# rubiruchi/ofdm_uhd

Hardware: AMD Instinct MI355X
Metric: OFDM symbols/sec (TX+loopback RX) @ N_fft=512; packet CRC pass rate (higher is better)
Workload: dtype f32; 1 GPU; N_fft=512, occ=200, QPSK, CP=128, synthetic AWGN channel (BASELINE configs[1]); payload_bytes=1026, symbols_per_packet=22, streams=1, iq_buffers=1, parallelism=independent streams, 1 per GPU

## Files before the change

include/ofdm_hip.h:

```cpp
#ifndef OFDM_HIP_H
#define OFDM_HIP_H

#include <stddef.h>
#include <stdint.h>

#ifdef __cplusplus
extern "C" {
#endif

#define OFDM_ABI_VERSION 6

#define OFDM_MAX_FFT 4096
#define OFDM_MAX_CARRIER_HEX 1024
#define OFDM_MAX_TAPS 512
#define OFDM_MAX_ARITY 256
#define OFDM_MASK_LEN 4096
#define OFDM_MAX_PKT_LEN 4096

enum {
  OFDM_OK = 0,
  OFDM_E_INVAL = -1,
  OFDM_E_NOMEM = -2,
  OFDM_E_CAPACITY = -3,
  OFDM_E_HIP = -4,
// ... 441 lines not shown
  OFDM_K_CHAN = 2,
  OFDM_K_SYNC = 3,
  OFDM_K_PEAK = 4,
  OFDM_K_DEMOD = 5,
  OFDM_K_DEFRAME = 6,
  OFDM_K_SENSE = 7,
  OFDM_K_FILTER = 8,
  OFDM_K_EXACT = 9,
  OFDM_K_FRONT = 10,
  OFDM_K_COUNT = 11
};
int ofdm_prof_enable(ofdm_handle *h, int on);
int ofdm_prof_reset(ofdm_handle *h);
int ofdm_prof_get(ofdm_handle *h, int kernel, double *total_ms, uint64_t *launches);
const char *ofdm_kernel_name(int kernel);

#ifdef __cplusplus
}
#endif
#endif
```

ofdm_uhd_amd/_abi.py:

```python
import ctypes as C
import os

OFDM_ABI_VERSION = 6
OFDM_MAX_FFT = 4096
OFDM_MAX_TAPS = 512
OFDM_MAX_ARITY = 256
OFDM_MASK_LEN = 4096
OFDM_MAX_PKT_LEN = 4096
OFDM_MAX_CARRIER_HEX = 1024
OFDM_DDC_MAX_TAPS = 1024
OFDM_DDC_BANK_MAX_LINKS = 8
OFDM_RESAMP_MAX_TAPS = 1024
OFDM_RESAMP_BANK_MAX_LINKS = 8
OFDM_DUC_MAX_TAPS = 1024
OFDM_DUC_BANK_MAX_LINKS = 8
OFDM_TX_RESAMP_MAX_TAPS = 1024
OFDM_TX_RESAMP_BANK_MAX_LINKS = 8
OFDM_PFB_MAX_CHANNELS = 64
OFDM_PFB_MAX_TAPS = 1024
OFDM_MULTIPATH_MAX_PATHS = 16
OFDM_MULTIPATH_MAX_TONES = 4
OFDM_MULTIPATH_MAX_DELAY = 1023
OFDM_FEC_MAX_PAYLOAD = 2040
OFDM_FEC_MAX_CODED = 4090
# ... 262 lines not shown
    ]


class ofdm_soft_cfg(C.Structure):
    _fields_ = [
        ("struct_size", C.c_uint32),
        ("scale", C.c_float),
    ]


EXPORTS = (
    "ofdm_abi_version", "ofdm_device_count", "ofdm_create", "ofdm_destroy", "ofdm_last_error",
    "ofdm_set_stream", "ofdm_set_tx_amplitude", "ofdm_set_carrier_map", "ofdm_set_channel", "ofdm_framed_len",
    "ofdm_make_packets", "ofdm_tx_frame_count", "ofdm_tx", "ofdm_tx_async", "ofdm_wait", "ofdm_channel", "ofdm_rx",
    "ofdm_set_taps", "ofdm_tap", "ofdm_prof_enable", "ofdm_prof_reset", "ofdm_prof_get",
    "ofdm_kernel_name", "ofdm_sense_count", "ofdm_sense", "ofdm_sense_decide", "ofdm_set_rx_sense",
    "ofdm_rx_sense_result", "ofdm_sense_device_msgs", "ofdm_sense_redecide",
    "ofdm_rx_packet_pos", "ofdm_rx_nco_state", "ofdm_rx_set_flag_history", "ofdm_rx_set_origin", "ofdm_rx_submit", "ofdm_rx_snr",
    "ofdm_set_rx_quality", "ofdm_rx_quality", "ofdm_set_rx_csi", "ofdm_rx_csi", "ofdm_rx_csi_summary",
    "ofdm_set_rx_iq_format", "ofdm_set_tx_iq_format",
    "ofdm_set_ddc", "ofdm_ddc_reset", "ofdm_ddc_count", "ofdm_ddc", "ofdm_ddc_taps", "ofdm_ddc_last_ms",
    "ofdm_set_duc", "ofdm_duc_reset", "ofdm_duc", "ofdm_duc_last_ms",
    "ofdm_set_ddc_bank", "ofdm_ddc_bank_reset", "ofdm_ddc_bank_count", "ofdm_ddc_bank", "ofdm_ddc_bank_taps",
    "ofdm_ddc_bank_last_ms",
    "ofdm_set_resamp", "ofdm_resamp_reset", "ofdm_resamp_count", "ofdm_resamp", "ofdm_resamp_taps", "ofdm_resamp_last_ms",
    "ofdm_set_resamp_bank", "ofdm_resamp_bank_reset", "ofdm_resamp_bank_count", "ofdm_resamp_bank", "ofdm_resamp_bank_taps",
    "ofdm_resamp_bank_last_ms",
    "ofdm_set_tx_resamp", "ofdm_tx_resamp_reset", "ofdm_tx_resamp_count", "ofdm_tx_resamp", "ofdm_tx_resamp_last_ms",
    "ofdm_set_pfb", "ofdm_pfb_reset", "ofdm_pfb_count", "ofdm_pfb", "ofdm_pfb_last_ms",
    "ofdm_set_pfb_synth", "ofdm_pfb_synth_reset", "ofdm_pfb_synth", "ofdm_pfb_synth_last_ms",
    "ofdm_set_duc_bank", "ofdm_duc_bank_reset", "ofdm_duc_bank", "ofdm_duc_bank_taps", "ofdm_duc_bank_last_ms",
# ... 101 lines not shown
    lib.ofdm_fec_last_ms.argtypes = [H, C.POINTER(C.c_double)]
    lib.ofdm_fec_coded_len_rate.argtypes = [C.c_uint32, C.c_uint32, u32p]
    lib.ofdm_fec_payload_len_rate.argtypes = [C.c_uint32, C.c_uint32, u32p]
    lib.ofdm_fec_punct_last_ms.argtypes = [H, C.POINTER(C.c_double)]
    lib.ofdm_set_rx_soft.argtypes = [H, C.POINTER(ofdm_soft_cfg)]
    lib.ofdm_rx_soft.argtypes = [H, vp, C.c_uint64, u64p, C.POINTER(C.c_int)]
    lib.ofdm_rx_fec_decode_soft.argtypes = [H, FC, u8p, C.c_uint64, u64p, vp, u32p, C.c_int, C.POINTER(C.c_int)]
    lib.ofdm_rx_soft_last_ms.argtypes = [H, C.POINTER(C.c_double)]
    lib.ofdm_set_taps.argtypes = [H, C.c_uint32]
    lib.ofdm_tap.argtypes = [H, C.c_int, vp, C.c_uint64, u64p]
    lib.ofdm_prof_enable.argtypes = [H, C.c_int]
    lib.ofdm_prof_reset.argtypes = [H]
    lib.ofdm_prof_get.argtypes = [H, C.c_int, C.POINTER(C.c_double), u64p]
    lib.ofdm_kernel_name.argtypes = [C.c_int]
    lib.ofdm_kernel_name.restype = C.c_char_p
    SC = C.POINTER(ofdm_sense_cfg)
    lib.ofdm_sense_count.argtypes = [SC, C.c_uint64, u64p, u64p]
    lib.ofdm_sense.argtypes = [H, SC, vp, C.c_uint64, vp, C.c_uint64, vp, vp, vp, C.c_uint64, u64p, u64p]
    lib.ofdm_sense_decide.argtypes = [H, SC, vp, C.c_uint64, vp, vp, vp, C.c_uint64, u64p]
    lib.ofdm_set_rx_sense.argtypes = [H, SC]
    lib.ofdm_rx_sense_result.argtypes = [H, vp, C.c_uint64, vp, vp, vp, C.c_uint64, u64p, u64p]
    lib.ofdm_rx_packet_pos.argtypes = [H, vp, C.c_int, C.POINTER(C.c_int)]
    lib.ofdm_rx_nco_state.argtypes = [H, vp, vp, vp, vp, C.c_int, C.POINTER(C.c_int)]
    lib.ofdm_rx_set_origin.argtypes = [H, C.c_uint64]
    lib.ofdm_rx_snr.argtypes = [H, C.POINTER(C.c_float)]
    lib.ofdm_set_rx_quality.argtypes = [H, C.c_int]
    lib.ofdm_rx_quality.argtypes = [H, vp, C.c_int, C.POINTER(C.c_int)]
    lib.ofdm_set_rx_csi.argtypes = [H, C.c_int]
    lib.ofdm_rx_csi.argtypes = [H, C.c_int, C.c_int, vp, vp, vp, vp, C.POINTER(C.c_int)]
    lib.ofdm_rx_csi_summary.argtypes = [H, C.c_int, u32p, vp, vp, vp, vp, vp]
# ... 39 lines not shown
```

ofdm_uhd_amd/csrc/engine.hip:

```cpp
#include <math.h>
#include <cmath>
#include <stdlib.h>
#include <string.h>

#include <algorithm>
#include <new>
#include <string>
#include <vector>

#include "common.h"
#include "fft.h"
#include "host_util.h"
#include "tx.h"
#include "rx_sync.h"
#include "rx_demod.h"
#include "rx_deframe.h"
#include "rx_soft.h"
#include "rx_state.h"
#include "sense.h"
#include "stream_hist.h"
#include "ddc.h"
#include "ddc_bank.h"
#include "duc.h"
#include "duc_bank.h"
// ... 287 lines not shown
  h->cfg.carrier_map[OFDM_MAX_CARRIER_HEX + 7] = 0;
  {
    int rc = apply_carrier_map(h, h->cfg.carrier_map);
    if (rc != OFDM_OK) return rc;
  }

  std::vector<c32> pre(N), tw(N);
  for (int i = 0; i < N; i++) pre[i] = c32{0.f, 0.f};
  for (int i = 0; i < occ; i++) {
    if (h->zl + i < N) pre[h->zl + i] = c32{cfg->known_symbol[i].re, cfg->known_symbol[i].im};
  }
  for (int k = 0; k < N; k++) {
    double a = -2.0 * M_PI * (double)k / (double)N;
    tw[k] = c32{(float)cos(a), (float)sin(a)};
  }
  uint32_t crc[256];
  for (uint32_t i = 0; i < 256; i++) {
    uint32_t c = i;
    for (int k = 0; k < 8; k++) c = (c & 1) ? (0xEDB88320u ^ (c >> 1)) : (c >> 1);
    crc[i] = c;
  }
  h->filtF = sync_filter_F((int)cfg->ntaps);
  std::vector<c32> Hf(h->filtF), twF(h->filtF);
  {
    const int F = h->filtF;
    std::vector<double> cs(F), sn(F);
    for (int m = 0; m < F; m++) {
      const double a = -2.0 * M_PI * (double)m / (double)F;
      cs[m] = cos(a);
      sn[m] = sin(a);
      twF[m] = c32{(float)cs[m], (float)sn[m]};
    }
    for (int k = 0; k < F; k++) {
      double re = 0.0, im = 0.0;
      for (int n = 0; n < (int)cfg->ntaps; n++) {
        const int idx = (int)(((long long)k * n) % F);
// ... 72 lines not shown
        if (seen & (1 << ix)) ok4 = false;
        seen |= 1 << ix;
        h->sign_idx[ix] = (unsigned char)i;
      }
      if (ok4) h->sign_kind = 2;
    }
    if (h->sign_kind) {
      const float lvl = h->sign_kind == 1 ? fabsf(c[0].re) : fminf(fabsf(c[0].re), fabsf(c[0].im));
      h->sign_eps = lvl * (1.0f / 512.0f);
      h->sign_bound = 8.0f * fmaxf(fabsf(c[0].re), fabsf(c[0].im));
    }
  }
  HIPCHK(h, upload(h->d_preamble, pre.data(), pre.size()));
  HIPCHK(h, upload(h->d_tw, tw.data(), tw.size()));
  HIPCHK(h, upload(h->d_mask, cfg->whitening_mask, (size_t)OFDM_MASK_LEN));
  HIPCHK(h, upload(h->d_crc, crc, (size_t)256));
  {
    std::vector<uint32_t> xp8(OFDM_MASK_LEN + 1);
    uint32_t v = 0x80000000u;
    for (size_t k = 0; k < xp8.size(); k++) {
      xp8[k] = v;
      for (int b = 0; b < 8; b++) v = (v & 1u) ? ((v >> 1) ^ 0xEDB88320u) : (v >> 1);
    }
    HIPCHK(h, upload(h->d_xp8, xp8.data(), xp8.size()));
  }
  {
    const double decay = (double)(1.0f - cfg->peak_alpha);
    std::vector<double> tab(2 * (SYNC_TILE + 1) + SYNC_THREADS / 2);
    double* dp = tab.data();
    double* ip = dp + (SYNC_TILE + 1);
    float* wt = reinterpret_cast<float*>(ip + (SYNC_TILE + 1));
// ... 495 lines not shown
```

ofdm_uhd_amd/csrc/engine_rx.inc:

```

template <typename T>
static int dev_excl_scan(ofdm_handle* h, const T* d_in, uint64_t n, T* d_out, T* d_total) {
  const uint64_t nb = (n + SCAN_BLOCK - 1) / SCAN_BLOCK;
  HIPCHK(h, h->rx.partial.ensure(sizeof(T) * std::max<uint64_t>(nb, 1)));
  T* part = h->rx.partial.as<T>();
  if (n == 0) {
    if (d_total) HIPCHK(h, hipMemsetAsync(d_total, 0, sizeof(T), h->stream));
    return OFDM_OK;
  }
  hipLaunchKernelGGL(HIP_KERNEL_NAME(k_scan_partials<T>), dim3((unsigned)nb), dim3(256), 0, h->stream, d_in, n, part);
  hipLaunchKernelGGL(HIP_KERNEL_NAME(k_scan_top<T>), dim3(1), dim3(256), 0, h->stream, part, nb, d_total);
  hipLaunchKernelGGL(HIP_KERNEL_NAME(k_scan_final<T>), dim3((unsigned)nb), dim3(256), 0, h->stream, d_in, n, part, d_out);
  HIPCHK(h, hipGetLastError());
  return OFDM_OK;
}

template <int N, bool TWL, bool TAPS, bool CSI = false>
static int launch_demod_t(ofdm_handle* h, const DemodParams& q, size_t shmem) {
  constexpr int T = N / 8, FPW = demod_fpw(N);
  if (shmem > 64 * 1024)
    HIPCHK(h, hipFuncSetAttribute(reinterpret_cast<const void*>(&k_rx_demod<N, TWL, TAPS, CSI>),
                                  hipFuncAttributeMaxDynamicSharedMemorySize, (int)shmem));
  hipLaunchKernelGGL(HIP_KERNEL_NAME(k_rx_demod<N, TWL, TAPS, CSI>), dim3((q.nframes + FPW - 1) / FPW), dim3(T * FPW), shmem,
                     h->stream, q);
// ... 38 lines not shown
}

static int run_demod(ofdm_handle* h, const DemodParams& q) {
  switch (h->N) {
    case 64: return launch_demod<64>(h, q);
    case 128: return launch_demod<128>(h, q);
    case 256: return launch_demod<256>(h, q);
    case 512: return launch_demod<512>(h, q);
    case 1024: return launch_demod<1024>(h, q);
    case 2048: return launch_demod<2048>(h, q);
    default: return launch_demod<4096>(h, q);
  }
}

enum { CT_CAND = 0, CT_OVERFLOW = 1, CT_NLO = 2, CT_NHI = 3, CT_CHAIN = 4, CT_NPEAKS = 5, CT_NSYM = 6, CT_KEYTOT = 7,
       CT_DEFR = 8 , CT_RAWTOT = 13, CT_PIECES = 14, CT_STASH = 15, CT_RECS = 16, CT_COUNT = 17 };

static int sync_params(ofdm_handle* h, uint64_t nsamples, bool cap_full, SyncParams* out) {
  RxState& rx = h->rx;
  const int N = h->N, CP = h->CP, T = SYNC_TILE;
  const uint64_t ntiles = (nsamples + T - 1) / T;
  const int tiles_per_seg = 32 * ((N + CP + T - 1) / T);
  const uint64_t egrid = std::min<uint64_t>(ntiles, 256ull * 8ull), egrid_small = std::min<uint64_t>(ntiles, 256ull * 16ull);
  const uint64_t cand_cap = (cap_full ? nsamples + nsamples / 8 : nsamples / 16) + (egrid + 16) * SYNC_CHUNK_C + egrid_small * 2048ull;
  const uint64_t piece_cap = (cap_full ? nsamples / 2 + 1 : nsamples / 128) + (egrid + egrid_small + 16) * SYNC_CHUNK_P;
  HIPCHK(h, rx.y.ensure(nsamples * sizeof(c32)));
  HIPCHK(h, rx.tile_B.ensure(ntiles * sizeof(double)));
  HIPCHK(h, rx.tile_np.ensure(ntiles * sizeof(uint32_t)));
  HIPCHK(h, rx.tile_pieces.ensure(piece_cap * sizeof(SyncPiece)));
  HIPCHK(h, rx.tile_first.ensure(ntiles * sizeof(uint64_t)));
  HIPCHK(h, rx.avg_in.ensure(ntiles * sizeof(double)));
  HIPCHK(h, rx.cand_u.ensure(cand_cap * sizeof(float)));
  HIPCHK(h, rx.cand_P.ensure(cand_cap * sizeof(c32)));
  HIPCHK(h, rx.counters.ensure(CT_COUNT * sizeof(uint64_t)));
  HIPCHK(h, rx.counts.ensure(ntiles * sizeof(uint32_t)));
  HIPCHK(h, rx.offsets.ensure(ntiles * sizeof(uint32_t)));
  HIPCHK(h, rx.recs.ensure(ntiles * sizeof(SyncRec)));
  float *d_metric = nullptr, *d_presel = nullptr;
  if (h->tap_mask & (1u << OFDM_TAP_RX_METRIC)) {
    HIPCHK(h, rx.metric.ensure(nsamples * sizeof(float)));
    d_metric = rx.metric.as<float>();
  }
  if (h->tap_mask & (1u << OFDM_TAP_RX_PRESEL)) {
    HIPCHK(h, rx.presel.ensure(nsamples * sizeof(float)));
    d_presel = rx.presel.as<float>();
  }
  uint64_t* ctr = rx.counters.as<uint64_t>();
  SyncParams sp;
  memset(&sp, 0, sizeof(sp));
  sp.N = N;
  sp.D = N / 2;
  sp.CP = CP;
// ... 293 lines not shown
static hipError_t launch_sync_exact(const void* fn, unsigned grid, size_t shmem, SyncParams sp, hipStream_t s) {
  void* args[] = {&sp};
  return hipLaunchKernel(fn, dim3(grid), dim3(SYNC_THREADS), args, shmem, s);
}

static int rx_sync_exact(RxCall& c, SyncParams& sp, bool cap_full) {
  ofdm_handle* h = c.h;
  if (cap_full) {
    int rcs = sync_params(h, c.nsamples, true, &sp);
    if (rcs != OFDM_OK) return rcs;
    uint64_t* ctr = rx_ctr(h);
    HIPCHK(h, hipMemsetAsync(ctr + CT_CAND, 0, 2 * sizeof(uint64_t), h->stream));
    HIPCHK(h, hipMemsetAsync(ctr + CT_NPEAKS, 0, sizeof(uint64_t), h->stream));
    HIPCHK(h, hipMemsetAsync(ctr + CT_PIECES, 0, 2 * sizeof(uint64_t), h->stream));
  }
  const unsigned egrid = (unsigned)std::min<uint64_t>(sp.ntiles, 256ull * 8ull);
  const unsigned egrid_small = (unsigned)std::min<uint64_t>(sp.ntiles, 256ull * 16ull);
  {
    ProfScope span(h->prof, OFDM_K_EXACT, h->stream);
    const size_t esh = exact_lds_layout(sp.CP, SYNC_TILE).total, esh_small = exact_lds_layout(sp.CP, sp.exact_small).total;
    const void* fbig = sp.D >= 2048 ? reinterpret_cast<const void*>(&k_sync_exact<SYNC_THREADS, true>)
                                    : reinterpret_cast<const void*>(&k_sync_exact<SYNC_THREADS, false>);
    if (esh > 64 * 1024) HIPCHK(h, hipFuncSetAttribute(fbig, hipFuncAttributeMaxDynamicSharedMemorySize, (int)esh));
    if (sp.exact_small > 0)
      hipLaunchKernelGGL(HIP_KERNEL_NAME(k_sync_exact<WAVE, false>), dim3(egrid_small), dim3(WAVE), esh_small, h->stream, sp);
    HIPCHK(h, launch_sync_exact(fbig, egrid, esh, sp, h->stream));
    if (sp.metric_tap) {
      SyncParams tp = sp;
      tp.tap_only = 1;
      HIPCHK(h, launch_sync_exact(fbig, egrid, esh, tp, h->stream));
    }
  }
  HIPCHK(h, hipGetLastError());
#ifdef SYNC_STAMPS
  if (!h->rx.front_done)
    if (int rs = sync_stamps_report(h, sp.stamps, sync_nseg(sp), sp.tiles_per_seg)) return rs;
#endif
  return OFDM_OK;
}

// ... 43 lines not shown
  HIPCHK(h, rx.stash_peaks.ensure(ntiles * PEAK_STASH * sizeof(uint64_t)));
  HIPCHK(h, rx.stash_P.ensure(ntiles * PEAK_STASH * sizeof(c32)));
  if (run_cap) HIPCHK(h, rx.run_rows.ensure(run_cap * 2 * sizeof(double)));
  PeakParams pp = make_peak_params(h, sp);
  hipLaunchKernelGGL(k_avg_carry, dim3(grid), dim3(256), 0, h->stream, rx.tile_B.as<double>(), ntiles, c.nsamples, sp.dpow,
                     rx.avg_in.as<double>());
  if (run_cap) HIPCHK(h, hipMemsetAsync(rx.run_rows.p, 0xFF, run_cap * 2 * sizeof(double), h->stream));
  hipLaunchKernelGGL(HIP_KERNEL_NAME(k_peak<false>), dim3(grid), dim3(256), 0, h->stream, pp);
  HIPCHK(h, hipGetLastError());
  int rc = dev_excl_scan<uint32_t>(h, rx.counts.as<uint32_t>(), ntiles, rx.offsets.as<uint32_t>(),
                                   reinterpret_cast<uint32_t*>(ctr + CT_NPEAKS));
  if (rc) return rc;
  uint64_t hc[CT_COUNT];
  HIPCHK(h, hipMemcpyAsync(hc, ctr, sizeof(hc), hipMemcpyDeviceToHost, h->stream));
  HIPCHK(h, hipStreamSynchronize(h->stream));
  if ((*overflow = hc[CT_OVERFLOW] & 0xFFFFFFFFull)) return OFDM_OK;
  rx.run_slots = std::min<uint64_t>(hc[CT_PIECES], run_cap);
  const uint64_t npeaks = hc[CT_NPEAKS] & 0xFFFFFFFFull;
  c.npeaks = rx.npeaks = npeaks;
  if (c.stats) c.stats->peaks = npeaks;
  if (npeaks == 0 && !(rx.nco_ref_on && !rx.hist_flags.empty())) {
    c.done = true;
    return OFDM_OK;
  }
  HIPCHK(h, rx.peaks.ensure(std::max<uint64_t>(npeaks, 1) * sizeof(uint64_t)));
  HIPCHK(h, rx.peak_P.ensure(std::max<uint64_t>(npeaks, 1) * sizeof(c32)));
  pp.peaks = rx.peaks.as<uint64_t>();
  pp.peak_P = rx.peak_P.as<c32>();
  if (npeaks > 0) {
    if (hc[CT_STASH] & 0xFFFFFFFFull)
// ... 793 lines not shown
  if (!peaks || !phi || !step || !swallowed || (uint64_t)cap < rx.npeaks) FAIL(h, OFDM_E_CAPACITY, "NCO state arrays too small");
  for (uint64_t i = 0; i < rx.npeaks; i++) swallowed[i] = i < rx.last_swallowed.size() ? rx.last_swallowed[i] : 0;
  HIPCHK(h, hipSetDevice(h->cfg.device_id));
  HIPCHK(h, hipMemcpy(peaks, rx.peaks.p, rx.npeaks * sizeof(uint64_t), hipMemcpyDeviceToHost));
  HIPCHK(h, hipMemcpy(phi, rx.Phi_u.p, rx.npeaks * sizeof(uint64_t), hipMemcpyDeviceToHost));
  HIPCHK(h, hipMemcpy(step, rx.step.p, rx.npeaks * sizeof(double), hipMemcpyDeviceToHost));
  return OFDM_OK;
}

extern "C" int ofdm_rx_snr(const ofdm_handle* h, float* snr_est) {
  if (!h || !snr_est) return OFDM_E_INVAL;
  *snr_est = 0.0f;
  return OFDM_OK;
}

extern "C" int ofdm_set_rx_quality(ofdm_handle* h, int enable) {
  if (!h) return OFDM_E_INVAL;
  h->rx.quality_on = enable != 0;
  return OFDM_OK;
}

extern "C" int ofdm_rx_quality(ofdm_handle* h, ofdm_pkt_quality* out, int cap, int* n) {
  if (!h) return OFDM_E_INVAL;
  const RxState& rx = h->rx;
  if (!rx.quality_valid) FAIL(h, OFDM_E_INVAL, "the last ofdm_rx ran without link quality (ofdm_set_rx_quality)");
  const size_t np = rx.last_quality.size();
  if (n) *n = (int)np;
  if (np == 0 || !out) return OFDM_OK;
  if ((size_t)cap < np) FAIL(h, OFDM_E_CAPACITY, "quality array too small");
  memcpy(out, rx.last_quality.data(), np * sizeof(ofdm_pkt_quality));
// ... 111 lines not shown
```

ofdm_uhd_amd/csrc/rx_deframe.h:

```cpp
#pragma once
#include "rx_demod.h"

__global__ void __launch_bounds__(256) k_chain_collect(const FrameResult* __restrict__ res, uint32_t nframes_s, DynFrames dyn,
                                                        uint32_t* __restrict__ list, uint32_t cap, unsigned int* count) {
  const uint32_t f = blockIdx.x * blockDim.x + threadIdx.x;
  const uint32_t nframes = dyn_nframes(dyn, nframes_s);
  if (f >= nframes) return;
  if (res[f].end_frame > f) {
    const unsigned int k = atomicAdd(count, 1u);
    if (k < cap) list[k] = f;
  }
}

__global__ void k_chain_resolve(const FrameResult* __restrict__ res, uint32_t nframes_s, DynFrames dyn, uint32_t* __restrict__ list,
                                uint32_t cap, const unsigned int* __restrict__ count, uint8_t* __restrict__ invalid,
                                unsigned int* overflow, const uint8_t* __restrict__ pre, uint32_t npre) {
  if (blockIdx.x != 0 || threadIdx.x != 0) return;
  const uint32_t nframes = dyn_nframes(dyn, nframes_s);
  for (uint32_t f = 0; f < npre && f < nframes; f++)
    if (pre[f]) invalid[f] = 1;
  unsigned int n = *count;
  if (n > cap) {
    int64_t cover = -1;
    for (uint32_t f = 0; f < nframes; f++) {
// ... 59 lines not shown
  }
  uint64_t key = 0;
  if (q.invalid[f]) {
    atomicAdd((unsigned long long*)&q.counters[3], 1ull);
  } else {
    const FrameResult r = q.res[f];
    if (r.header_ok) atomicAdd((unsigned long long*)&q.counters[0], 1ull);
    if (r.status == FR_COMPLETE) {
      const uint64_t plen = r.packetlen >= 4 ? r.packetlen - 4 : 0;
      key = (1ull << 40) | plen;
    }
  }
  q.key[f] = key;
}

__global__ void __launch_bounds__(256) k_deframe_write(DeframeParams q) {
  __shared__ uint32_t tab[256];
  __shared__ __align__(16) uint32_t stage_all[4][260];
  tab[threadIdx.x] = q.crc_table[threadIdx.x];
  __syncthreads();
  const int lane = lane_id(), w = wave_id();
  uint32_t* stage = stage_all[w];
  const uint32_t f = blockIdx.x * 4 + (uint32_t)w;
  if (f >= dyn_nframes(q.dyn, q.nframes)) return;
  if (q.invalid[f]) return;
  const FrameResult r = q.res[f];
  if (r.status != FR_COMPLETE) return;
  const uint64_t pos = q.pos[f];
  const uint64_t ord = pos >> 40, boff = pos & ((1ull << 40) - 1);
  const uint32_t len = r.packetlen;
  const uint32_t plen = len >= 4 ? len - 4 : 0;
  if (ord >= q.max_pkts || boff + plen > q.payload_cap) {
    if (lane == 0) atomicAdd((unsigned long long*)&q.counters[4], 1ull);
    return;
  }
  const uint8_t* msg = q.raw + (uint64_t)f * RAW_SLOT;
  const uint4* msg4 = reinterpret_cast<const uint4*>(msg);
  const uint4* mask4 = reinterpret_cast<const uint4*>(q.mask);
  uint8_t* out = q.payload_out + boff;
  uint32_t acc = 0;
  for (uint32_t c0 = 0; c0 < plen; c0 += 1024) {
    const uint32_t o = c0 + 16u * (uint32_t)lane;
    uint4 d = make_uint4(0, 0, 0, 0);
    if (o < plen) {
      const uint4 m = msg4[o >> 4], k = mask4[o >> 4];
      d = make_uint4(m.x ^ k.x, m.y ^ k.y, m.z ^ k.z, m.w ^ k.w);
      const uint32_t nb = (plen - o < 16u) ? (plen - o) : 16u;
      uint32_t crc = 0xFFFFFFFFu;
      const uint32_t wds[4] = {d.x, d.y, d.z, d.w};
#pragma unroll
      for (int b = 0; b < 16; b++) {
        if ((uint32_t)b < nb) {
          const uint32_t byte = (wds[b >> 2] >> (8 * (b & 3))) & 0xFFu;
          crc = tab[(crc ^ byte) & 0xFF] ^ (crc >> 8);
        }
      }
      crc ^= 0xFFFFFFFFu;
      acc ^= crc_multmodp(q.xp8[plen - (o + nb)], crc);
    }
    reinterpret_cast<uint4*>(stage)[lane] = d;
    if (lane == 0) stage[256] = 0;
    __builtin_amdgcn_wave_barrier();
    __builtin_amdgcn_s_waitcnt(0xC07F);
    const uint32_t rem = (plen - c0 < 1024u) ? (plen - c0) : 1024u;
    uint8_t* og = out + c0;
    const uint32_t head0 = (4u - (uint32_t)((uintptr_t)og & 3u)) & 3u;
    const uint32_t head = head0 < rem ? head0 : rem;
    const uint32_t nd = (rem - head) >> 2;
    const uint8_t* st8 = reinterpret_cast<const uint8_t*>(stage);
    if ((uint32_t)lane < head) og[lane] = st8[lane];
    for (uint32_t dw = (uint32_t)lane; dw < nd; dw += WAVE) {
      const uint32_t i0 = head + 4u * dw;
      const uint32_t w0 = stage[i0 >> 2], w1 = stage[(i0 >> 2) + 1];
      reinterpret_cast<uint32_t*>(og + i0)[0] = __builtin_amdgcn_alignbyte(w1, w0, i0 & 3u);
    }
    const uint32_t tail0 = head + 4u * nd;
    if (tail0 + (uint32_t)lane < rem) og[tail0 + lane] = st8[tail0 + lane];
    __builtin_amdgcn_wave_barrier();
  }
#pragma unroll
  for (int d = WAVE / 2; d > 0; d >>= 1) acc ^= __shfl_xor(acc, d, WAVE);
  if (lane == 0) {
    int ok = 0;
    if (len >= 4) {
      const uint32_t got = ((uint32_t)(msg[plen] ^ q.mask[plen]) << 24) | ((uint32_t)(msg[plen + 1] ^ q.mask[plen + 1]) << 16) |
                           ((uint32_t)(msg[plen + 2] ^ q.mask[plen + 2]) << 8) | (uint32_t)(msg[plen + 3] ^ q.mask[plen + 3]);
      ok = (acc == got);
    }
    q.out_off[ord] = boff;
    q.out_len[ord] = plen;
    q.out_ok[ord] = (uint8_t)ok;
    q.out_pos[ord] = q.peaks[dyn_j0(q.dyn, q.j0) + f];
  }
// ... 174 lines not shown
```

ofdm_uhd_amd/csrc/rx_state.h:

```cpp
#pragma once
#include "host_util.h"
#include "rx_demod.h"

#define RX_DEVBUFS(X)                                                                                                       \
  X(recs) X(x_stage) X(y) X(metric) X(presel) X(tile_B) X(tile_np) X(tile_first) X(tile_pieces) X(avg_in) X(cand_u)        \
  X(cand_P) X(counters) X(counts) X(offsets) X(partial) X(peaks) X(peak_P) X(angle) X(step) X(inc) X(Phi) X(K) X(nsym)     \
  X(sym_base) X(res) X(raw) X(invalid) X(chain_list) X(key) X(pos) X(out_payload) X(out_off) X(out_len) X(out_ok)          \
  X(out_pos) X(inc_acc) X(Phi_u) X(peaks2) X(peak_P2) X(fstep) X(pre_inv) X(stash_peaks) X(stash_P) X(tap_fft) X(tap_acq)  \
  X(tap_sink) X(tap_demapped) X(raw_tap) X(raw_lens) X(raw_pos) X(tap_sampler) X(tap_sigmix) X(tap_nco) X(qual_frame)      \
  X(qual_out) X(csi_frame) X(csi_rows) X(csi_part) X(csi_sum) X(run_rows) X(soft_vals)

struct RxState {
#define X(name) DevBuf name;
  RX_DEVBUFS(X)
#undef X
  uint64_t nsamples = 0, npeaks = 0, nframes = 0, j0 = 0, nsym_total = 0, raw_tap_bytes = 0;
  uint64_t run_slots = 0;
  const c32* y_ptr = nullptr;
  bool sub_valid = false, in_event_at_end = false;
  bool front_done = false;
  bool sub_hold = false;
  const void* sub_iq = nullptr;
  uint64_t sub_n = 0;
  const c32* sub_dx = nullptr;
  uint64_t origin = 0;
  std::vector<uint64_t> last_pos;
  bool nco_ref_on = false;
  int64_t nco_ref_peak = 0, nco_trust_after = 0;
  uint64_t nco_ref_u = 0;
  double nco_ref_step = 0.0;
  std::vector<uint64_t> hist_flags;
  std::vector<double> hist_steps;
// ... 25 lines not shown
```

ofdm_uhd_amd/csrc/rx_sync.h:

```cpp
#pragma once
#include "common.h"
#include "fft.h"

#ifndef SYNC_THREADS
#define SYNC_THREADS 256
#endif
#define SYNC_V 8
#define SYNC_TILE (SYNC_THREADS * SYNC_V)
#define SYNC_GUARD 1.0e-3f
#define SYNC_ILL 0.015625f
#define SYNC_CHUNK_C 4096
#ifndef SYNC_MAX_WG
#define SYNC_MAX_WG 5
#endif
#define SYNC_CHUNK_P 1024

struct SyncPiece {
  uint64_t start;
  uint64_t end;
  uint64_t val_off;
  double bloc;
};

struct SyncRec {
// ... 22 lines not shown
  const double* dpow;
  const double* ipow;
  const float* wtab;
  double* tile_B;
  uint32_t* tile_npieces;
  uint64_t* tile_first;
  SyncPiece* pieces;
  uint64_t piece_cap;
  unsigned long long* piece_count;
  float* cand_u;
  c32* cand_P;
  uint64_t cand_cap;
  unsigned long long* cand_count;
  unsigned int* overflow;
  int exact_small;
  SyncRec* recs;
  unsigned long long* rec_count;
};

__host__ __device__ inline int sync_lp(int i) { return i + (i >> 3); }

__host__ __device__ inline int sync_filter_F(int ntaps) {
  int p2 = 1;
  while (p2 < ntaps) p2 <<= 1;
  const int f = 2 * p2;
  return f < 64 ? 64 : f;
}
__host__ __device__ inline int sync_ring_samples(int HY) { return (HY + SYNC_TILE + 7) / 8 * 8; }

struct FilterParams {
  int B;
  int ntm1;
  int goff;
// ... 501 lines not shown
#endif

#ifdef SYNC_DIAG
#define SYNC_ABLATE(p, bit) ((p).ablate & (bit))
#else
#define SYNC_ABLATE(p, bit) 0
#endif
__device__ __forceinline__ bool sync_tile_ill(const float* slots, uint64_t tile) {
  constexpr int NW = SYNC_THREADS / WAVE;
  const float* sl = slots + (int)(tile & 1u) * NW * 6;
  bool ill = false;
#pragma unroll
  for (int w = 0; w < NW; w++) ill = ill || reinterpret_cast<const int*>(sl + 6 * w)[5] != 0;
  return ill;
}
__device__ __forceinline__ bool sync_finish_tile(const SyncParams& p, const float* slots, uint64_t tile, bool prev_ill) {
  constexpr int NW = SYNC_THREADS / WAVE;
  const float* sl = slots + (int)(tile & 1u) * NW * 6;
  const bool ill = sync_tile_ill(slots, tile);
  if (ill || prev_ill) {
    const uint64_t t0 = tile * (uint64_t)SYNC_TILE;
    const unsigned long long r = atomicAdd(p.rec_count, 1ull);
    SyncRec rec;
    rec.tile = tile;
    rec.amin = 0;
    rec.bmax = ((t0 + (uint64_t)SYNC_TILE <= p.nsamples) ? SYNC_TILE : (int)(p.nsamples - t0)) - 1;
    rec.gpre = rec.gpost = 0.0f;
    p.recs[r] = rec;
    return ill;
  }
  int w0 = -1, w1 = -1;
#pragma unroll
  for (int w = 0; w < NW; w++) {
    if (reinterpret_cast<const int*>(sl + 6 * w)[4] >= 0) {
      if (w0 < 0) w0 = w;
      w1 = w;
    }
  }
  if (w0 < 0) {
    float tb = sl[0];
    if (NW == 4) tb = (sl[0] + sl[6]) + (sl[12] + sl[18]);
    else if (NW == 2) tb = sl[0] + sl[6];
    p.tile_B[tile] = (double)tb;
    p.tile_npieces[tile] = 0;
    return ill;
  }
  float ga = 0.f, gb = 0.f;
#pragma unroll
  for (int w = 0; w < NW; w++) {
    ga += (w < w0) ? sl[6 * w] : (w == w0) ? sl[6 * w + 1] : 0.0f;
    gb += (w > w1) ? sl[6 * w] : (w == w1) ? sl[6 * w + 2] : 0.0f;
  }
  const unsigned long long r = atomicAdd(p.rec_count, 1ull);
  SyncRec rec;
  rec.tile = tile;
  rec.amin = reinterpret_cast<const int*>(sl + 6 * w0)[3];
  rec.bmax = reinterpret_cast<const int*>(sl + 6 * w1)[4];
  rec.gpre = ga;
  rec.gpost = gb;
  p.recs[r] = rec;
  return ill;
}

template <int W, bool STATIC, int F = 0>
__global__ void __launch_bounds__(SYNC_THREADS, W) k_sync(SyncParams p, FilterParams fp) {
#ifdef SYNC_STAMPS
  unsigned long long st_acc[16] = {0, 0, 0, 0, 0, 0, 0, 0, 0, 0, 0, 0, 0, 0, 0, 0};
  unsigned long long st_last = __builtin_amdgcn_s_memtime();
#endif
  constexpr bool FUSED = F > 0;
  static_assert(!FUSED || (STATIC && F <= 512), "the fused front end uses the fixed LDS layout and wave-sized transforms");
  extern __shared__ __align__(16) unsigned char smem[];
  const int tid = threadIdx.x;
  constexpr int T = SYNC_TILE;
  const int R = p.R;
// ... 388 lines not shown
}
template <int NT, bool KEEP>
__global__ void __launch_bounds__(NT) k_sync_exact(SyncParams p) {
  extern __shared__ __align__(16) unsigned char smem[];
  constexpr int T = SYNC_TILE;
  constexpr bool SMALL = NT == WAVE;
  constexpr unsigned CHUNK_C = SMALL ? 2048u : (unsigned)SYNC_CHUNK_C;
  const int tl = threadIdx.x;
  const ExactLds L = exact_lds_layout(p.CP, SMALL ? p.exact_small : T);
  float* me = reinterpret_cast<float*>(smem + L.me);
  float* ue = reinterpret_cast<float*>(smem + L.ue);
  unsigned char* misc = smem + L.misc;
  long long* sc_i64 = reinterpret_cast<long long*>(misc);
  unsigned long long* bc = reinterpret_cast<unsigned long long*>(misc + 320);
  const int D = p.D, CP = p.CP;
  const unsigned long long nrec = p.tap_only ? (unsigned long long)p.ntiles : *p.rec_count;
  unsigned long long cand_base = 0, piece_base = 0;
  uint32_t cand_left = 0, piece_left = 0;
  const double alpha_d = (double)p.alpha;

  for (unsigned long long ri = blockIdx.x; ri < nrec; ri += gridDim.x) {
    SyncRec rec;
    if (p.tap_only) {
      rec.tile = ri;
      rec.amin = 0;
      const uint64_t left = p.nsamples - ri * (uint64_t)T;
      rec.bmax = (left < (uint64_t)T ? (int)left : T) - 1;
      rec.gpre = rec.gpost = 0.f;
    } else {
      rec = p.recs[ri];
    }
    const uint64_t tile = rec.tile;
    const int amin = rec.amin, bmax = rec.bmax;
    if (!p.tap_only && (bmax - amin + 1 <= p.exact_small) != SMALL) continue;
    const uint64_t t0 = tile * (uint64_t)T;
    const int64_t t0s = (int64_t)t0;
    const int Tl = (t0 + (uint64_t)T <= p.nsamples) ? T : (int)(p.nsamples - t0);
    const int rlen = bmax - amin + 1;

    if (p.tap_only) {
      sync_exact_range<NT, KEEP>(p.y, me, ue, nullptr, p.metric_tap + t0 + (uint64_t)amin, sc_i64, amin, bmax, D, CP, t0s, p.tapcp);
      continue;
    }

    if ((uint32_t)rlen > cand_left) {
      if (tl == 0) bc[0] = atomicAdd(p.cand_count, (unsigned long long)CHUNK_C);
      __syncthreads();
      cand_base = bc[0];
      cand_left = CHUNK_C;
// ... 280 lines not shown
```

ofdm_uhd_amd/engine.py:

```python
import ctypes as C
import importlib

import numpy as np

from . import _abi, config, iqio


def _quality_dtype():
    st = _abi.ofdm_pkt_quality
    conv = {C.c_uint64: np.uint64, C.c_uint32: np.uint32, C.c_int32: np.int32, C.c_float: np.float32}
    return np.dtype({"names": [f for f, _ in st._fields_],
                     "formats": [conv[t] for _, t in st._fields_],
                     "offsets": [getattr(st, f).offset for f, _ in st._fields_],
                     "itemsize": C.sizeof(st)})


QUALITY_DTYPE = _quality_dtype()


class EngineError(RuntimeError):
    def __init__(self, code, msg):
        RuntimeError.__init__(self, "libofdm_hip: %s (code %d)" % (msg, code))
        self.code = code

# ... 112 lines not shown
    def prof_enable(self, on=True):
        self._check(self._lib.ofdm_prof_enable(self._h, 1 if on else 0))

    def prof_reset(self):
        self._check(self._lib.ofdm_prof_reset(self._h))

    def prof(self):
        out = {}
        for k in range(_abi.K_COUNT):
            ms = C.c_double(0)
            n = C.c_uint64(0)
            self._check(self._lib.ofdm_prof_get(self._h, k, C.byref(ms), C.byref(n)))
            out[self._lib.ofdm_kernel_name(k).decode()] = (ms.value, n.value)
        return out

    def framed_len(self, payload_len):
        n = C.c_uint32(0)
        self._check(self._lib.ofdm_framed_len(self._h, int(payload_len), C.byref(n)))
        return n.value

    def make_packets(self, payloads):
        assert not self.device_ptrs
        blob, offs, lens = pack_payloads(payloads)
        total = 0
        for ln in lens:
            total += self.framed_len(int(ln))
        out = np.zeros(max(total, 1), np.uint8)
        foff = np.zeros(len(payloads) + 1, np.uint64)
        self._check(self._lib.ofdm_make_packets(self._h, _ptr(blob), offs.ctypes.data_as(C.POINTER(C.c_uint64)),
                                                lens.ctypes.data_as(C.POINTER(C.c_uint32)), len(payloads), _ptr(out),
# ... 716 lines not shown
```

Baseline: 132.0 million OFDM symbols/s.

## Split sync exact records by size class and use slicing-by-4 CRC

Sync tile records are now appended into two per-class lists (small and big range), each with its own counter. Each k_sync_exact launch therefore iterates only over its own class instead of scanning all records and skipping the rest. The deframe CRC switches from byte-at-a-time table lookups to a slicing-by-4 table in shared memory, and a short final chunk is handled by a dedicated tail path. The cost is doubled record storage, a larger CRC table upload and LDS footprint, and a new query API for per-class counts.

Result: no change. 132.8 million OFDM symbols/s, median of 5 (+0.6%).

```diff
diff --git a/include/ofdm_hip.h b/include/ofdm_hip.h
--- a/include/ofdm_hip.h
+++ b/include/ofdm_hip.h
@@ -479,6 +479,7 @@
 int ofdm_prof_reset(ofdm_handle *h);
 int ofdm_prof_get(ofdm_handle *h, int kernel, double *total_ms, uint64_t *launches);
 const char *ofdm_kernel_name(int kernel);
+int ofdm_rx_exact_records(const ofdm_handle *h, uint64_t counts[2]);
 
 #ifdef __cplusplus
 }
diff --git a/ofdm_uhd_amd/_abi.py b/ofdm_uhd_amd/_abi.py
--- a/ofdm_uhd_amd/_abi.py
+++ b/ofdm_uhd_amd/_abi.py
@@ -300,7 +300,7 @@
     "ofdm_set_stream", "ofdm_set_tx_amplitude", "ofdm_set_carrier_map", "ofdm_set_channel", "ofdm_framed_len",
     "ofdm_make_packets", "ofdm_tx_frame_count", "ofdm_tx", "ofdm_tx_async", "ofdm_wait", "ofdm_channel", "ofdm_rx",
     "ofdm_set_taps", "ofdm_tap", "ofdm_prof_enable", "ofdm_prof_reset", "ofdm_prof_get",
-    "ofdm_kernel_name", "ofdm_sense_count", "ofdm_sense", "ofdm_sense_decide", "ofdm_set_rx_sense",
+    "ofdm_kernel_name", "ofdm_rx_exact_records", "ofdm_sense_count", "ofdm_sense", "ofdm_sense_decide", "ofdm_set_rx_sense",
     "ofdm_rx_sense_result", "ofdm_sense_device_msgs", "ofdm_sense_redecide",
     "ofdm_rx_packet_pos", "ofdm_rx_nco_state", "ofdm_rx_set_flag_history", "ofdm_rx_set_origin", "ofdm_rx_submit", "ofdm_rx_snr",
     "ofdm_set_rx_quality", "ofdm_rx_quality", "ofdm_set_rx_csi", "ofdm_rx_csi", "ofdm_rx_csi_summary",
@@ -432,6 +432,7 @@
     lib.ofdm_prof_get.argtypes = [H, C.c_int, C.POINTER(C.c_double), u64p]
     lib.ofdm_kernel_name.argtypes = [C.c_int]
     lib.ofdm_kernel_name.restype = C.c_char_p
+    lib.ofdm_rx_exact_records.argtypes = [H, u64p]
     SC = C.POINTER(ofdm_sense_cfg)
     lib.ofdm_sense_count.argtypes = [SC, C.c_uint64, u64p, u64p]
     lib.ofdm_sense.argtypes = [H, SC, vp, C.c_uint64, vp, C.c_uint64, vp, vp, vp, C.c_uint64, u64p, u64p]
diff --git a/ofdm_uhd_amd/csrc/engine.hip b/ofdm_uhd_amd/csrc/engine.hip
--- a/ofdm_uhd_amd/csrc/engine.hip
+++ b/ofdm_uhd_amd/csrc/engine.hip
@@ -325,12 +325,17 @@
     double a = -2.0 * M_PI * (double)k / (double)N;
     tw[k] = c32{(float)cos(a), (float)sin(a)};
   }
-  uint32_t crc[256];
+  uint32_t crc[4 * 256];
   for (uint32_t i = 0; i < 256; i++) {
     uint32_t c = i;
     for (int k = 0; k < 8; k++) c = (c & 1) ? (0xEDB88320u ^ (c >> 1)) : (c >> 1);
     crc[i] = c;
   }
+  for (uint32_t k = 1; k < 4; k++)
+    for (uint32_t i = 0; i < 256; i++) {
+      const uint32_t c = crc[256 * (k - 1) + i];
+      crc[256 * k + i] = (c >> 8) ^ crc[c & 0xFFu];
+    }
   h->filtF = sync_filter_F((int)cfg->ntaps);
   std::vector<c32> Hf(h->filtF), twF(h->filtF);
   {
@@ -433,7 +438,7 @@
   HIPCHK(h, upload(h->d_preamble, pre.data(), pre.size()));
   HIPCHK(h, upload(h->d_tw, tw.data(), tw.size()));
   HIPCHK(h, upload(h->d_mask, cfg->whitening_mask, (size_t)OFDM_MASK_LEN));
-  HIPCHK(h, upload(h->d_crc, crc, (size_t)256));
+  HIPCHK(h, upload(h->d_crc, crc, (size_t)(4 * 256)));
   {
     std::vector<uint32_t> xp8(OFDM_MASK_LEN + 1);
     uint32_t v = 0x80000000u;
diff --git a/ofdm_uhd_amd/csrc/engine_rx.inc b/ofdm_uhd_amd/csrc/engine_rx.inc
--- a/ofdm_uhd_amd/csrc/engine_rx.inc
+++ b/ofdm_uhd_amd/csrc/engine_rx.inc
@@ -76,14 +76,17 @@
 }
 
 enum { CT_CAND = 0, CT_OVERFLOW = 1, CT_NLO = 2, CT_NHI = 3, CT_CHAIN = 4, CT_NPEAKS = 5, CT_NSYM = 6, CT_KEYTOT = 7,
-       CT_DEFR = 8 , CT_RAWTOT = 13, CT_PIECES = 14, CT_STASH = 15, CT_RECS = 16, CT_COUNT = 17 };
+       CT_DEFR = 8 , CT_RAWTOT = 13, CT_PIECES = 14, CT_STASH = 15, CT_RECS = 16 , CT_COUNT = 18 };
+static_assert(CT_RECS + EXACT_CLASSES == CT_COUNT, "one record counter per k_sync_exact class");
+
+static uint64_t sync_exact_grid(uint64_t ntiles, int cls) { return std::min<uint64_t>(ntiles, cls == EXACT_BIG ? 256ull * 8ull : 256ull * 16ull); }
 
 static int sync_params(ofdm_handle* h, uint64_t nsamples, bool cap_full, SyncParams* out) {
   RxState& rx = h->rx;
   const int N = h->N, CP = h->CP, T = SYNC_TILE;
   const uint64_t ntiles = (nsamples + T - 1) / T;
   const int tiles_per_seg = 32 * ((N + CP + T - 1) / T);
-  const uint64_t egrid = std::min<uint64_t>(ntiles, 256ull * 8ull), egrid_small = std::min<uint64_t>(ntiles, 256ull * 16ull);
+  const uint64_t egrid = sync_exact_grid(ntiles, EXACT_BIG), egrid_small = sync_exact_grid(ntiles, EXACT_SMALL);
   const uint64_t cand_cap = (cap_full ? nsamples + nsamples / 8 : nsamples / 16) + (egrid + 16) * SYNC_CHUNK_C + egrid_small * 2048ull;
   const uint64_t piece_cap = (cap_full ? nsamples / 2 + 1 : nsamples / 128) + (egrid + egrid_small + 16) * SYNC_CHUNK_P;
   HIPCHK(h, rx.y.ensure(nsamples * sizeof(c32)));
@@ -97,7 +100,7 @@
   HIPCHK(h, rx.counters.ensure(CT_COUNT * sizeof(uint64_t)));
   HIPCHK(h, rx.counts.ensure(ntiles * sizeof(uint32_t)));
   HIPCHK(h, rx.offsets.ensure(ntiles * sizeof(uint32_t)));
-  HIPCHK(h, rx.recs.ensure(ntiles * sizeof(SyncRec)));
+  HIPCHK(h, rx.recs.ensure(EXACT_CLASSES * ntiles * sizeof(SyncRec)));
   float *d_metric = nullptr, *d_presel = nullptr;
   if (h->tap_mask & (1u << OFDM_TAP_RX_METRIC)) {
     HIPCHK(h, rx.metric.ensure(nsamples * sizeof(float)));
@@ -421,16 +424,19 @@
     HIPCHK(h, hipMemsetAsync(ctr + CT_NPEAKS, 0, sizeof(uint64_t), h->stream));
     HIPCHK(h, hipMemsetAsync(ctr + CT_PIECES, 0, 2 * sizeof(uint64_t), h->stream));
   }
-  const unsigned egrid = (unsigned)std::min<uint64_t>(sp.ntiles, 256ull * 8ull);
-  const unsigned egrid_small = (unsigned)std::min<uint64_t>(sp.ntiles, 256ull * 16ull);
+  const unsigned egrid = (unsigned)sync_exact_grid(sp.ntiles, EXACT_BIG);
   {
     ProfScope span(h->prof, OFDM_K_EXACT, h->stream);
-    const size_t esh = exact_lds_layout(sp.CP, SYNC_TILE).total, esh_small = exact_lds_layout(sp.CP, sp.exact_small).total;
+    const size_t esh = exact_lds_layout(sp.CP, SYNC_TILE).total;
     const void* fbig = sp.D >= 2048 ? reinterpret_cast<const void*>(&k_sync_exact<SYNC_THREADS, true>)
                                     : reinterpret_cast<const void*>(&k_sync_exact<SYNC_THREADS, false>);
     if (esh > 64 * 1024) HIPCHK(h, hipFuncSetAttribute(fbig, hipFuncAttributeMaxDynamicSharedMemorySize, (int)esh));
-    if (sp.exact_small > 0)
-      hipLaunchKernelGGL(HIP_KERNEL_NAME(k_sync_exact<WAVE, false>), dim3(egrid_small), dim3(WAVE), esh_small, h->stream, sp);
+    if (sp.exact_small > 0) {
+      sp.exact_class = EXACT_SMALL;
+      hipLaunchKernelGGL(HIP_KERNEL_NAME(k_sync_exact<WAVE, false>), dim3((unsigned)sync_exact_grid(sp.ntiles, EXACT_SMALL)), dim3(WAVE),
+                         exact_lds_layout(sp.CP, sp.exact_small).total, h->stream, sp);
+    }
+    sp.exact_class = EXACT_BIG;
     HIPCHK(h, launch_sync_exact(fbig, egrid, esh, sp, h->stream));
     if (sp.metric_tap) {
       SyncParams tp = sp;
@@ -504,6 +510,7 @@
   uint64_t hc[CT_COUNT];
   HIPCHK(h, hipMemcpyAsync(hc, ctr, sizeof(hc), hipMemcpyDeviceToHost, h->stream));
   HIPCHK(h, hipStreamSynchronize(h->stream));
+  for (int k = 0; k < EXACT_CLASSES; k++) rx.exact_recs[k] = hc[CT_RECS + k];
   if ((*overflow = hc[CT_OVERFLOW] & 0xFFFFFFFFull)) return OFDM_OK;
   rx.run_slots = std::min<uint64_t>(hc[CT_PIECES], run_cap);
   const uint64_t npeaks = hc[CT_NPEAKS] & 0xFFFFFFFFull;
@@ -1327,6 +1334,12 @@
   return OFDM_OK;
 }
 
+extern "C" int ofdm_rx_exact_records(const ofdm_handle* h, uint64_t counts[2]) {
+  if (!h || !counts) return OFDM_E_INVAL;
+  for (int k = 0; k < EXACT_CLASSES; k++) counts[k] = h->rx.exact_recs[k];
+  return OFDM_OK;
+}
+
 extern "C" int ofdm_set_rx_quality(ofdm_handle* h, int enable) {
   if (!h) return OFDM_E_INVAL;
   h->rx.quality_on = enable != 0;
diff --git a/ofdm_uhd_amd/csrc/rx_deframe.h b/ofdm_uhd_amd/csrc/rx_deframe.h
--- a/ofdm_uhd_amd/csrc/rx_deframe.h
+++ b/ofdm_uhd_amd/csrc/rx_deframe.h
@@ -97,10 +97,27 @@
   q.key[f] = key;
 }
 
+__device__ __forceinline__ uint32_t crc32_piece16(const uint32_t (*tab)[256], const uint32_t wds[4], uint32_t nb) {
+  uint32_t crc = 0xFFFFFFFFu;
+#pragma unroll
+  for (int w = 0; w < 4; w++) {
+    if (4u * (uint32_t)w + 4u <= nb) {
+      const uint32_t c = crc ^ wds[w];
+      crc = tab[3][c & 0xFFu] ^ tab[2][(c >> 8) & 0xFFu] ^ tab[1][(c >> 16) & 0xFFu] ^ tab[0][c >> 24];
+    } else {
+#pragma unroll
+      for (int b = 0; b < 4; b++)
+        if ((uint32_t)(4 * w + b) < nb) crc = tab[0][(crc ^ (wds[w] >> (8 * b))) & 0xFFu] ^ (crc >> 8);
+    }
+  }
+  return crc ^ 0xFFFFFFFFu;
+}
+
 __global__ void __launch_bounds__(256) k_deframe_write(DeframeParams q) {
-  __shared__ uint32_t tab[256];
+  __shared__ uint32_t tab[4][256];
   __shared__ __align__(16) uint32_t stage_all[4][260];
-  tab[threadIdx.x] = q.crc_table[threadIdx.x];
+#pragma unroll
+  for (int k = 0; k < 4; k++) tab[k][threadIdx.x] = q.crc_table[256 * k + threadIdx.x];
   __syncthreads();
   const int lane = lane_id(), w = wave_id();
   uint32_t* stage = stage_all[w];
@@ -122,24 +139,16 @@
   const uint4* mask4 = reinterpret_cast<const uint4*>(q.mask);
   uint8_t* out = q.payload_out + boff;
   uint32_t acc = 0;
-  for (uint32_t c0 = 0; c0 < plen; c0 += 1024) {
+  uint32_t c0 = 0;
+  for (; c0 < plen && plen - c0 > 16u; c0 += 1024) {
     const uint32_t o = c0 + 16u * (uint32_t)lane;
     uint4 d = make_uint4(0, 0, 0, 0);
     if (o < plen) {
       const uint4 m = msg4[o >> 4], k = mask4[o >> 4];
       d = make_uint4(m.x ^ k.x, m.y ^ k.y, m.z ^ k.z, m.w ^ k.w);
       const uint32_t nb = (plen - o < 16u) ? (plen - o) : 16u;
-      uint32_t crc = 0xFFFFFFFFu;
       const uint32_t wds[4] = {d.x, d.y, d.z, d.w};
-#pragma unroll
-      for (int b = 0; b < 16; b++) {
-        if ((uint32_t)b < nb) {
-          const uint32_t byte = (wds[b >> 2] >> (8 * (b & 3))) & 0xFFu;
-          crc = tab[(crc ^ byte) & 0xFF] ^ (crc >> 8);
-        }
-      }
-      crc ^= 0xFFFFFFFFu;
-      acc ^= crc_multmodp(q.xp8[plen - (o + nb)], crc);
+      acc ^= crc_multmodp(q.xp8[plen - (o + nb)], crc32_piece16(tab, wds, nb));
     }
     reinterpret_cast<uint4*>(stage)[lane] = d;
     if (lane == 0) stage[256] = 0;
@@ -160,6 +169,16 @@
     const uint32_t tail0 = head + 4u * nd;
     if (tail0 + (uint32_t)lane < rem) og[tail0 + lane] = st8[tail0 + lane];
     __builtin_amdgcn_wave_barrier();
+  }
+  if (c0 < plen) {
+    const uint32_t nb = plen - c0;
+    const uint4 m = msg4[c0 >> 4], k = mask4[c0 >> 4];
+    const uint32_t wds[4] = {m.x ^ k.x, m.y ^ k.y, m.z ^ k.z, m.w ^ k.w};
+    if (lane == 0) acc ^= crc32_piece16(tab, wds, nb);
+    if ((uint32_t)lane < nb) {
+      const uint32_t wl = (lane & 8) ? ((lane & 4) ? wds[3] : wds[2]) : ((lane & 4) ? wds[1] : wds[0]);
+      out[c0 + (uint32_t)lane] = (uint8_t)(wl >> (8 * (lane & 3)));
+    }
   }
 #pragma unroll
   for (int d = WAVE / 2; d > 0; d >>= 1) acc ^= __shfl_xor(acc, d, WAVE);
diff --git a/ofdm_uhd_amd/csrc/rx_state.h b/ofdm_uhd_amd/csrc/rx_state.h
--- a/ofdm_uhd_amd/csrc/rx_state.h
+++ b/ofdm_uhd_amd/csrc/rx_state.h
@@ -16,6 +16,7 @@
 #undef X
   uint64_t nsamples = 0, npeaks = 0, nframes = 0, j0 = 0, nsym_total = 0, raw_tap_bytes = 0;
   uint64_t run_slots = 0;
+  uint64_t exact_recs[2] = {0, 0};
   const c32* y_ptr = nullptr;
   bool sub_valid = false, in_event_at_end = false;
   bool front_done = false;
diff --git a/ofdm_uhd_amd/csrc/rx_sync.h b/ofdm_uhd_amd/csrc/rx_sync.h
--- a/ofdm_uhd_amd/csrc/rx_sync.h
+++ b/ofdm_uhd_amd/csrc/rx_sync.h
@@ -60,9 +60,12 @@
   unsigned long long* cand_count;
   unsigned int* overflow;
   int exact_small;
+  int exact_class;
   SyncRec* recs;
   unsigned long long* rec_count;
 };
+enum { EXACT_SMALL = 0, EXACT_BIG = 1, EXACT_CLASSES = 2 };
+__host__ __device__ inline int sync_exact_class(int rlen, int exact_small) { return rlen <= exact_small ? EXACT_SMALL : EXACT_BIG; }
 
 __host__ __device__ inline int sync_lp(int i) { return i + (i >> 3); }
 
@@ -594,19 +597,23 @@
   for (int w = 0; w < NW; w++) ill = ill || reinterpret_cast<const int*>(sl + 6 * w)[5] != 0;
   return ill;
 }
+__device__ __forceinline__ void sync_append_rec(const SyncParams& p, const SyncRec& rec) {
+  const int cls = sync_exact_class(rec.bmax - rec.amin + 1, p.exact_small);
+  const unsigned long long r = atomicAdd(p.rec_count + cls, 1ull);
+  p.recs[(unsigned long long)cls * p.ntiles + r] = rec;
+}
 __device__ __forceinline__ bool sync_finish_tile(const SyncParams& p, const float* slots, uint64_t tile, bool prev_ill) {
   constexpr int NW = SYNC_THREADS / WAVE;
   const float* sl = slots + (int)(tile & 1u) * NW * 6;
   const bool ill = sync_tile_ill(slots, tile);
   if (ill || prev_ill) {
     const uint64_t t0 = tile * (uint64_t)SYNC_TILE;
-    const unsigned long long r = atomicAdd(p.rec_count, 1ull);
     SyncRec rec;
     rec.tile = tile;
     rec.amin = 0;
     rec.bmax = ((t0 + (uint64_t)SYNC_TILE <= p.nsamples) ? SYNC_TILE : (int)(p.nsamples - t0)) - 1;
     rec.gpre = rec.gpost = 0.0f;
-    p.recs[r] = rec;
+    sync_append_rec(p, rec);
     return ill;
   }
   int w0 = -1, w1 = -1;
@@ -631,14 +638,13 @@
     ga += (w < w0) ? sl[6 * w] : (w == w0) ? sl[6 * w + 1] : 0.0f;
     gb += (w > w1) ? sl[6 * w] : (w == w1) ? sl[6 * w + 2] : 0.0f;
   }
-  const unsigned long long r = atomicAdd(p.rec_count, 1ull);
   SyncRec rec;
   rec.tile = tile;
   rec.amin = reinterpret_cast<const int*>(sl + 6 * w0)[3];
   rec.bmax = reinterpret_cast<const int*>(sl + 6 * w1)[4];
   rec.gpre = ga;
   rec.gpost = gb;
-  p.recs[r] = rec;
+  sync_append_rec(p, rec);
   return ill;
 }
 
@@ -1057,7 +1063,8 @@
   long long* sc_i64 = reinterpret_cast<long long*>(misc);
   unsigned long long* bc = reinterpret_cast<unsigned long long*>(misc + 320);
   const int D = p.D, CP = p.CP;
-  const unsigned long long nrec = p.tap_only ? (unsigned long long)p.ntiles : *p.rec_count;
+  const unsigned long long nrec = p.tap_only ? (unsigned long long)p.ntiles : p.rec_count[p.exact_class];
+  const SyncRec* recs = p.recs + (unsigned long long)p.exact_class * p.ntiles;
   unsigned long long cand_base = 0, piece_base = 0;
   uint32_t cand_left = 0, piece_left = 0;
   const double alpha_d = (double)p.alpha;
@@ -1071,11 +1078,10 @@
       rec.bmax = (left < (uint64_t)T ? (int)left : T) - 1;
       rec.gpre = rec.gpost = 0.f;
     } else {
-      rec = p.recs[ri];
+      rec = recs[ri];
     }
     const uint64_t tile = rec.tile;
     const int amin = rec.amin, bmax = rec.bmax;
-    if (!p.tap_only && (bmax - amin + 1 <= p.exact_small) != SMALL) continue;
     const uint64_t t0 = tile * (uint64_t)T;
     const int64_t t0s = (int64_t)t0;
     const int Tl = (t0 + (uint64_t)T <= p.nsamples) ? T : (int)(p.nsamples - t0);
diff --git a/ofdm_uhd_amd/engine.py b/ofdm_uhd_amd/engine.py
--- a/ofdm_uhd_amd/engine.py
+++ b/ofdm_uhd_amd/engine.py
@@ -150,6 +150,11 @@
             out[self._lib.ofdm_kernel_name(k).decode()] = (ms.value, n.value)
         return out
 
+    def rx_exact_records(self):
+        n = (C.c_uint64 * 2)()
+        self._check(self._lib.ofdm_rx_exact_records(self._h, n))
+        return tuple(int(v) for v in n)
+
     def framed_len(self, payload_len):
         n = C.c_uint32(0)
         self._check(self._lib.ofdm_framed_len(self._h, int(payload_len), C.byref(n)))
```
